# arpg/vicalib

Hardware: AMD Instinct MI355X
Metric: corner_residuals_per_sec (higher is better)
Workload: dtype f64

## Files before the change

### vicalib_amd/csrc/vc_imu.hpp

```cpp
#pragma once
#include "vc_math.hpp"

namespace vc {

struct D1 { double a, v; };
VC_HD D1 mk(double a, double v = 0.0) { D1 r; r.a = a; r.v = v; return r; }
VC_HD D1 operator+(D1 x, D1 y) { return mk(x.a + y.a, x.v + y.v); }
VC_HD D1 operator-(D1 x, D1 y) { return mk(x.a - y.a, x.v - y.v); }
VC_HD D1 operator-(D1 x) { return mk(-x.a, -x.v); }
VC_HD D1 operator*(D1 x, D1 y) { return mk(x.a * y.a, x.a * y.v + x.v * y.a); }
VC_HD D1 operator/(D1 x, D1 y) { const double inv = fast_rcp(y.a), q = x.a * inv; return mk(q, (x.v - q * y.v) * inv); }
VC_HD D1 operator+(D1 x, double s) { return mk(x.a + s, x.v); }
VC_HD D1 operator+(double s, D1 x) { return mk(x.a + s, x.v); }
VC_HD D1 operator-(D1 x, double s) { return mk(x.a - s, x.v); }
VC_HD D1 operator-(double s, D1 x) { return mk(s - x.a, -x.v); }
VC_HD D1 operator*(D1 x, double s) { return mk(x.a * s, x.v * s); }
VC_HD D1 operator*(double s, D1 x) { return mk(x.a * s, x.v * s); }
VC_HD D1 operator/(D1 x, double s) { const double inv = 1.0 / s; return mk(x.a * inv, x.v * inv); }
VC_HD D1 operator/(double s, D1 y) { const double inv = fast_rcp(y.a); return mk(s * inv, -s * inv * inv * y.v); }
VC_HD bool operator<(D1 x, double y) { return x.a < y; }
VC_HD bool operator>(D1 x, double y) { return x.a > y; }
VC_HD D1 sqrt(D1 x) { double s, is; fast_sqrt_rsqrt(x.a, &s, &is); return mk(s, 0.5 * x.v * is); }
VC_HD D1 sin(D1 x) { return mk(::sin(x.a), ::cos(x.a) * x.v); }
VC_HD D1 cos(D1 x) { return mk(::cos(x.a), -::sin(x.a) * x.v); }
// ... 304 lines not shown
  J[0 * 6 + 3] = 0.5 * q0; J[0 * 6 + 4] = -0.5 * q3; J[0 * 6 + 5] = 0.5 * q2;
  J[1 * 6 + 3] = 0.5 * q3; J[1 * 6 + 4] = 0.5 * q0; J[1 * 6 + 5] = -0.5 * q1;
  J[2 * 6 + 3] = -0.5 * q2; J[2 * 6 + 4] = 0.5 * q1; J[2 * 6 + 5] = 0.5 * q0;
  J[3 * 6 + 3] = -0.5 * q1; J[3 * 6 + 4] = -0.5 * q2; J[3 * 6 + 5] = -0.5 * q3;
  J[4 * 6 + 0] = 1.0 - 2.0 * (q2 * q2 + q3 * q3); J[4 * 6 + 1] = 2.0 * (q1 * q2 - q0 * q3); J[4 * 6 + 2] = 2.0 * (q1 * q3 + q0 * q2);
  J[5 * 6 + 0] = 2.0 * (q1 * q2 + q0 * q3); J[5 * 6 + 1] = 1.0 - 2.0 * (q1 * q1 + q3 * q3); J[5 * 6 + 2] = 2.0 * (q2 * q3 - q0 * q1);
  J[6 * 6 + 0] = 2.0 * (q1 * q3 - q0 * q2); J[6 * 6 + 1] = 2.0 * (q2 * q3 + q0 * q1); J[6 * 6 + 2] = 1.0 - 2.0 * (q1 * q1 + q2 * q2);
}

VC_HD void imu_block_direction(const ImuView& buf, double t_start, double t_end, const double* w_sqrt, int rotation_only,
                               const double* T2, const double* T1, const double* v2, const double* v1, const double* gdir,
                               const double* b, const double* sf, double toff, int dir, double* r, double* dr) {
  D1 P[35];
  for (int i = 0; i < 7; ++i) { P[i] = mk(T2[i]); P[7 + i] = mk(T1[i]); }
  for (int i = 0; i < 3; ++i) { P[14 + i] = mk(v2[i]); P[17 + i] = mk(v1[i]); }
  P[20] = mk(gdir[0]); P[21] = mk(gdir[1]);
  for (int i = 0; i < 6; ++i) { P[22 + i] = mk(b[i]); P[28 + i] = mk(sf[i]); }
  P[34] = mk(toff);
  for (int i = 0; i < 35; ++i) P[i].v = (i == dir) ? 1.0 : 0.0;
  D1 res[9];
  imu_residual<D1>(buf, t_start, t_end, w_sqrt, rotation_only, P, P + 7, P + 14, P + 17, P + 20, P + 22, P + 28, P[34], res);
  for (int i = 0; i < 9; ++i) { r[i] = res[i].a; dr[i] = res[i].v; }
}

constexpr int kDeltaCols = 14;

template <class T> struct DeltaAcc { T q[4], p[3], v[3], t; };
template <class T> VC_HD void imu_delta_append(DeltaAcc<T>* A, const PoseV<T>& d, T dt) {
  T rp[3], rv[3], q[4];
  tq_rotate(A->q, d.p, rp);
  tq_rotate(A->q, d.v, rv);
  tq_mul(A->q, d.q, q);
  for (int i = 0; i < 3; ++i) {
    A->p[i] = (A->p[i] + A->v[i] * dt) + rp[i];
    A->v[i] = A->v[i] + rv[i];
  }
  for (int i = 0; i < 4; ++i) A->q[i] = q[i];
  A->t = A->t + dt;
}
template <class T> VC_HD void imu_delta_then(DeltaAcc<T>* a, const DeltaAcc<T>& x) {
  PoseV<T> d;
  for (int k = 0; k < 4; ++k) d.q[k] = x.q[k];
  for (int k = 0; k < 3; ++k) { d.p[k] = x.p[k]; d.v[k] = x.v[k]; }
  imu_delta_append(a, d, x.t);
}
template <class T> VC_HD void imu_delta_identity(DeltaAcc<T>* a) {
  for (int k = 0; k < 3; ++k) { a->q[k] = cst<T>(0.0); a->p[k] = cst<T>(0.0); a->v[k] = cst<T>(0.0); }
  a->q[3] = cst<T>(1.0); a->t = cst<T>(0.0);
}
constexpr int kBlockDeltaStride = kDeltaCols * 11;

VC_HD void so3_exp_jl(const double* w, double* q, double* A, double* B) {
  const double th2 = w[0] * w[0] + w[1] * w[1] + w[2] * w[2];
  double imag, real;
  tso3_exp_factors(th2, &imag, &real);
  q[0] = imag * w[0]; q[1] = imag * w[1]; q[2] = imag * w[2]; q[3] = real;
  const bool tiny = th2 < 1e-6;
  *A = 2.0 * imag * imag;
  *B = tiny ? 1.0 / 6.0 - th2 * (1.0 / 120.0) : (1.0 - 2.0 * imag * real) * fast_rcp(tiny ? 1.0 : th2);
}
VC_HD void cross3(const double* a, const double* b, double* o) {
  const double x = a[1] * b[2] - a[2] * b[1], y = a[2] * b[0] - a[0] * b[2], z = a[0] * b[1] - a[1] * b[0];
  o[0] = x; o[1] = y; o[2] = z;
}
VC_HD void so3_jl_apply(const double* w, double A, double B, const double* d, double* o) {
  double c1[3], c2[3];
  cross3(w, d, c1);
  cross3(w, c1, c2);
  for (int i = 0; i < 3; ++i) o[i] = d[i] + A * c1[i] + B * c2[i];
}
VC_HD void mat3_vec(const double* R, const double* v, double* o) {
  const double a = R[0] * v[0] + R[1] * v[1] + R[2] * v[2];
  const double b = R[3] * v[0] + R[4] * v[1] + R[5] * v[2];
  const double c = R[6] * v[0] + R[7] * v[1] + R[8] * v[2];
  o[0] = a; o[1] = b; o[2] = c;
}
struct IntervalDeltaT { DeltaAcc<double> d; double dth[3], dp[3], dv[3], dt; double ap[3], av[3]; };
constexpr int kDtDoubles = 27;
VC_HD void imu_delta_t_identity(IntervalDeltaT* X) {
  imu_delta_identity(&X->d);
  for (int i = 0; i < 3; ++i) { X->dth[i] = 0.0; X->dp[i] = 0.0; X->dv[i] = 0.0; X->ap[i] = 0.0; X->av[i] = 0.0; }
  X->dt = 0.0;
}
VC_HD void imu_interval_delta_t(const ImuView& buf, const ImuRange& rg, D1 off, double t_start, double t_end, int m, int n_int,
                                const double* b, const double* sf, int gsel, IntervalDeltaT* X) {
  imu_delta_t_identity(X);
  const int kk = gsel < 3 ? gsel : (gsel < 6 ? gsel - 3 : 0);
  const bool seeded = gsel < 6, scale = gsel >= 3;
  double u0[3], u1[3], a0[3], a1[3], du0[3], du1[3], da0[3], da1[3], h, dh;
  double c0, c1;
  {
    Meas<D1> z0, z1;
    for (int k = 0; k < 3; ++k) { z0.w[k] = z0.a[k] = z1.w[k] = z1.a[k] = mk(0.0); }
    z0.time = z1.time = mk(0.0);
    if (m <= n_int) { imu_range_get_flat(buf, rg, off, t_start, t_end, m - 1, &z0); imu_range_get_flat(buf, rg, off, t_start, t_end, m, &z1); }
    if (z1.time.a == z0.time.a) return;
    h = z1.time.a - z0.time.a; dh = z1.time.v - z0.time.v;
    for (int i = 0; i < 3; ++i) {
      const double s0 = (seeded && i == kk) ? (scale ? z0.w[i].a : 1.0) : 0.0, s1 = (seeded && i == kk) ? (scale ? z1.w[i].a : 1.0) : 0.0;
      u0[i] = z0.w[i].a * sf[i] + b[i]; du0[i] = z0.w[i].v * sf[i] + s0;
      u1[i] = z1.w[i].a * sf[i] + b[i]; du1[i] = z1.w[i].v * sf[i] + s1;
      a0[i] = z0.a[i].a * sf[3 + i] + b[3 + i]; da0[i] = z0.a[i].v * sf[3 + i];
      a1[i] = z1.a[i].a * sf[3 + i] + b[3 + i]; da1[i] = z1.a[i].v * sf[3 + i];
    }
    c0 = scale ? (kk == 0 ? z0.a[0].a : kk == 1 ? z0.a[1].a : z0.a[2].a) : 1.0;
    c1 = scale ? (kk == 0 ? z1.a[0].a : kk == 1 ? z1.a[1].a : z1.a[2].a) : 1.0;
  }
  const double hh = h * 0.5, h6 = h / 6.0, dhh = dh * 0.5, dh6 = dh / 6.0;
  const double cm = 0.5 * c0 + 0.5 * c1;
  double sw[3], sv[3], sp[3], dsw[3], dsv[3], dsp[3], cv[3], cp[3], phi[3], dphi[3];
  for (int i = 0; i < 3; ++i) {
    sw[i] = u0[i]; dsw[i] = du0[i]; sv[i] = a0[i]; dsv[i] = da0[i]; sp[i] = a0[i]; dsp[i] = da0[i];
    cv[i] = (i == kk) ? c0 : 0.0; cp[i] = cv[i];
    phi[i] = u0[i] * hh; dphi[i] = du0[i] * hh + u0[i] * dhh;
  }
  for (int stage = 2; stage <= 4; ++stage) {
    double q[4], A, B, R[9], dth[3], ug[3], ua[3], dug[3], dua[3], wk[3], ak[3], dwk[3], dak[3], t1[3], t2[3];
    so3_exp_jl(phi, q, &A, &B);
    quat_to_R(q, R);
    so3_jl_apply(phi, A, B, dphi, dth);
    for (int i = 0; i < 3; ++i) {
      if (stage < 4) { ug[i] = u0[i] * 0.5 + u1[i] * 0.5; ua[i] = a0[i] * 0.5 + a1[i] * 0.5; dug[i] = du0[i] * 0.5 + du1[i] * 0.5; dua[i] = da0[i] * 0.5 + da1[i] * 0.5; }
      else { ug[i] = u1[i]; ua[i] = a1[i]; dug[i] = du1[i]; dua[i] = da1[i]; }
    }
    mat3_vec(R, ug, wk); mat3_vec(R, ua, ak);
    cross3(dth, wk, t1); mat3_vec(R, dug, t2);
    for (int i = 0; i < 3; ++i) dwk[i] = t1[i] + t2[i];
    cross3(dth, ak, t1); mat3_vec(R, dua, t2);
    for (int i = 0; i < 3; ++i) dak[i] = t1[i] + t2[i];
    const double r[3] = {kk == 0 ? R[0] : kk == 1 ? R[1] : R[2], kk == 0 ? R[3] : kk == 1 ? R[4] : R[5], kk == 0 ? R[6] : kk == 1 ? R[7] : R[8]};
    const double wgt = stage < 4 ? 2.0 : 1.0, cc = stage < 4 ? cm : c1;
    for (int i = 0; i < 3; ++i) {
      sw[i] = sw[i] + wgt * wk[i]; dsw[i] = dsw[i] + wgt * dwk[i];
      sv[i] = sv[i] + wgt * ak[i]; dsv[i] = dsv[i] + wgt * dak[i];
      cv[i] = cv[i] + wgt * (cc * r[i]);
      if (stage < 4) { sp[i] = sp[i] + ak[i]; dsp[i] = dsp[i] + dak[i]; cp[i] = cp[i] + cc * r[i]; }
      const double hs = stage == 2 ? hh : h, dhs = stage == 2 ? dhh : dh;
      if (stage < 4) { phi[i] = wk[i] * hs; dphi[i] = dwk[i] * hs + wk[i] * dhs; }
    }
  }
  {
    double A, B;
    for (int i = 0; i < 3; ++i) { phi[i] = sw[i] * h6; dphi[i] = dsw[i] * h6 + sw[i] * dh6; }
    so3_exp_jl(phi, X->d.q, &A, &B);
    so3_jl_apply(phi, A, B, dphi, X->dth);
    const double hh6 = h * h6, dhh6 = 2.0 * h * dh6;
    for (int i = 0; i < 3; ++i) {
      X->d.v[i] = sv[i] * h6; X->dv[i] = dsv[i] * h6 + sv[i] * dh6;
      X->d.p[i] = sp[i] * hh6; X->dp[i] = dsp[i] * hh6 + sp[i] * dhh6;
      X->av[i] = cv[i] * h6; X->ap[i] = cp[i] * hh6;
    }
    X->d.t = h; X->dt = dh;
  }
}
VC_HD void imu_delta_t_then(IntervalDeltaT* A, const IntervalDeltaT& X) {
  double R[9], rp[3], rv[3], t1[3], t2[3], t3[3], q[4];
  quat_to_R(A->d.q, R);
  mat3_vec(R, X.d.p, rp); mat3_vec(R, X.d.v, rv);
  cross3(A->dth, rp, t1); mat3_vec(R, X.dp, t2);
  for (int i = 0; i < 3; ++i) A->dp[i] = ((A->dp[i] + A->dv[i] * X.d.t) + A->d.v[i] * X.dt) + (t1[i] + t2[i]);
  cross3(A->dth, rv, t1); mat3_vec(R, X.dv, t2);
  for (int i = 0; i < 3; ++i) A->dv[i] = A->dv[i] + (t1[i] + t2[i]);
  mat3_vec(R, X.dth, t3);
  for (int i = 0; i < 3; ++i) A->dth[i] = A->dth[i] + t3[i];
  A->dt = A->dt + X.dt;
  mat3_vec(R, X.ap, t1); mat3_vec(R, X.av, t2);
  for (int i = 0; i < 3; ++i) {
    A->ap[i] = (A->ap[i] + A->av[i] * X.d.t) + t1[i];
    A->av[i] = A->av[i] + t2[i];
  }
  for (int i = 0; i < 3; ++i) {
    A->d.p[i] = (A->d.p[i] + A->d.v[i] * X.d.t) + rp[i];
    A->d.v[i] = A->d.v[i] + rv[i];
  }
  quat_mul(A->d.q, X.d.q, q);
  for (int i = 0; i < 4; ++i) A->d.q[i] = q[i];
  A->d.t = A->d.t + X.d.t;
}
VC_HD int imu_group_dual_col(int g) { return g < 3 ? 1 + g : (g < 6 ? 4 + g : 13); }
VC_HD int imu_group_accel_col(int g) { return g < 3 ? 4 + g : 7 + g; }
VC_HD void imu_block_record_store(const IntervalDeltaT& X, int g, double* rec) {
  if (g > 6) return;
  double* cd = rec + imu_group_dual_col(g) * 11;
  const double hq[4] = {0.5 * X.dth[0], 0.5 * X.dth[1], 0.5 * X.dth[2], 0.0};
  double dq[4];
  quat_mul(hq, X.d.q, dq);
  for (int k = 0; k < 4; ++k) cd[k] = dq[k];
  for (int k = 0; k < 3; ++k) { cd[4 + k] = X.dp[k]; cd[7 + k] = X.dv[k]; }
  cd[10] = X.dt;
  if (g < 6) {
    double* ca = rec + imu_group_accel_col(g) * 11;
    for (int k = 0; k < 4; ++k) ca[k] = 0.0;
    for (int k = 0; k < 3; ++k) { ca[4 + k] = X.ap[k]; ca[7 + k] = X.av[k]; }
    ca[10] = 0.0;
  }
  if (g == 0) {
    for (int k = 0; k < 4; ++k) rec[k] = X.d.q[k];
    for (int k = 0; k < 3; ++k) { rec[4 + k] = X.d.p[k]; rec[7 + k] = X.d.v[k]; }
    rec[10] = X.d.t;
  }
}
inline int imu_block_delta_record(const ImuView& buf, double t_start, double t_end, double toff, const double* b, const double* sf,
                                  double* rec ) {
  const ImuRange rg = imu_range(buf, t_start, t_end, toff);
  if (!rg.valid) { rec[10] = -1.0; return 0; }
  const int n_int = (rg.k1 - rg.k0 + 1) + 1;
  for (int g = 0; g < 7; ++g) {
    const D1 offD = mk(toff, g == 6 ? 1.0 : 0.0);
    IntervalDeltaT carry;
    for (int base = 0; base < n_int; base += 16) {
      IntervalDeltaT X[8], Y[8];
      for (int l = 0; l < 8; ++l) {
        IntervalDeltaT second;
        imu_interval_delta_t(buf, rg, offD, t_start, t_end, base + 2 * l + 1, n_int, b, sf, g, &X[l]);
        imu_interval_delta_t(buf, rg, offD, t_start, t_end, base + 2 * l + 2, n_int, b, sf, g, &second);
        imu_delta_t_then(&X[l], second);
      }
      for (int n = 1; n < 8; n <<= 1) {
        for (int l = 0; l < 8; ++l) { Y[l] = X[l]; if (l >= n) { Y[l] = X[l - n]; imu_delta_t_then(&Y[l], X[l]); } }
        for (int l = 0; l < 8; ++l) X[l] = Y[l];
      }
      if (base == 0) carry = X[7]; else imu_delta_t_then(&carry, X[7]);
    }
    imu_block_record_store(carry, g, rec);
  }
  return 1;
}

VC_HD void imu_block_final_direction(int valid, const double* block_rec, const double* w_sqrt, int rotation_only, const double* T2,
                                     const double* T1, const double* v2, const double* v1, const double* grav9 , int col,
                                     double* r, double* dr) {
  if (!valid) { for (int i = 0; i < 9; ++i) { r[i] = 0.0; dr[i] = 0.0; } return; }
  const int dcol = (col >= 20) ? col - 19 : 0;
  D1 Q[4], P[3], V[3];
  double bd[11];
  for (int k = 0; k < 11; ++k) { const double d = block_rec[dcol * 11 + k]; bd[k] = dcol ? d : 0.0; }
  for (int k = 0; k < 4; ++k) Q[k] = mk(block_rec[k], bd[k]);
  for (int k = 0; k < 3; ++k) { P[k] = mk(block_rec[4 + k], bd[4 + k]); V[k] = mk(block_rec[7 + k], bd[7 + k]); }
  const D1 Tt = mk(block_rec[10], bd[10]);
  D1 T2D[7], v2D[3], gw[3], q0[4], p0[3], v0[3];
  {
    double J[42];
    local_jac_se3(T2, J);
    for (int i = 0; i < 7; ++i) {
      double sel = 0.0;
      for (int c = 0; c < 6; ++c) sel = (col == c) ? J[i * 6 + c] : sel;
      T2D[i] = mk(T2[i], sel);
    }
    local_jac_se3(T1, J);
    for (int i = 0; i < 7; ++i) {
      double sel = 0.0;
      for (int c = 0; c < 6; ++c) sel = (col == 9 + c) ? J[i * 6 + c] : sel;
      if (i < 4) q0[i] = mk(T1[i], sel); else p0[i - 4] = mk(T1[i], sel);
    }
  }
  for (int k = 0; k < 3; ++k) { v2D[k] = mk(v2[k], col == 6 + k ? 1.0 : 0.0); v0[k] = mk(v1[k], col == 15 + k ? 1.0 : 0.0); }
  for (int k = 0; k < 3; ++k) gw[k] = mk(grav9[k], col == 18 ? grav9[3 + k] : (col == 19 ? grav9[6 + k] : 0.0));
  PoseV<D1> x;
  D1 rp[3], rv[3];
  tq_rotate(q0, P, rp);
  tq_rotate(q0, V, rv);
  tq_mul(q0, Q, x.q);
  const D1 ht2 = 0.5 * (Tt * Tt);
  for (int i = 0; i < 3; ++i) {
    x.p[i] = ((p0[i] + v0[i] * Tt) - gw[i] * ht2) + rp[i];
    x.v[i] = (v0[i] - gw[i] * Tt) + rv[i];
  }
  D1 res[9];
  imu_residual_tail(x, w_sqrt, rotation_only, T2D, v2D, res);
  for (int i = 0; i < 9; ++i) { r[i] = res[i].a; dr[i] = res[i].v; }
}

}
```

### vicalib_amd/csrc/vc_imu_kernels.hip

```cpp
#include <hip/hip_runtime.h>
#include <algorithm>
#include <cstdlib>
#include "vc_math.hpp"
#include "vc_imu.hpp"
#include "vc_imu_weights.hpp"
#include "vc_device.h"
#include "vc_kutil.hpp"
#include "vc_reduced_tail.hpp"
#include "vc_shared_blocks.hpp"

namespace vc {

__device__ __forceinline__ ImuView imu_view(const DevView& v) { ImuView b = {v.imu_t, v.imu_w, v.imu_a, v.n_imu, v.imu_avg_dt}; return b; }

constexpr int kImuJacLds = 34 * 9 + 6;
struct SegTab {
  unsigned short v[kSegStride];
  constexpr SegTab() : v() { for (int e = 0; e < kSegLen; ++e) { int a = 0, b = 0; seg_entry(e, &a, &b); v[e] = (unsigned short)(a | (b << 8)); } }
};
__constant__ SegTab d_seg_tab = SegTab();
constexpr int kSegIters = (kSegLen + 31) / 32;
#ifndef VC_IJ_MFMA
#define VC_IJ_MFMA 1
#endif
// ... 182 lines not shown
#pragma unroll
  for (int e = 0; e < N; ++e) x[e] += y[e];
}
template <int N> __device__ __forceinline__ void row_allsum_n(double* x) {
  row_add_level<0xB1, N>(x);
  row_add_level<0x4E, N>(x);
  row_add_level<0x141, N>(x);
  row_add_level<0x140, N>(x);
}
__device__ __forceinline__ double shfl16(double x, int src) { return __shfl(x, src, 16); }
__device__ __forceinline__ void delta_identity(DeltaAcc<double>* a) {
#pragma unroll
  for (int k = 0; k < 3; ++k) { a->q[k] = 0.0; a->p[k] = 0.0; a->v[k] = 0.0; }
  a->q[3] = 1.0; a->t = 0.0;
}
__device__ __forceinline__ void delta_then(DeltaAcc<double>* a, const DeltaAcc<double>& x) {
  PoseV<double> d;
#pragma unroll
  for (int k = 0; k < 4; ++k) d.q[k] = x.q[k];
#pragma unroll
  for (int k = 0; k < 3; ++k) { d.p[k] = x.p[k]; d.v[k] = x.v[k]; }
  imu_delta_append(a, d, x.t);
}
template <int N> __device__ __forceinline__ void delta_scan_level(DeltaAcc<double>* X, int c) {
  DeltaAcc<double> A;
#pragma unroll
  for (int k = 0; k < 4; ++k) A.q[k] = row_shr<N>(X->q[k], X->q[k]);
#pragma unroll
  for (int k = 0; k < 3; ++k) { A.p[k] = row_shr<N>(X->p[k], X->p[k]); A.v[k] = row_shr<N>(X->v[k], X->v[k]); }
  A.t = row_shr<N>(X->t, X->t);
  delta_then(&A, *X);
  if (c >= N) *X = A;
}
template <int N> __device__ __forceinline__ void map_scan_level(double* S) {
  double B[kWMapF], O[kWMapF];
  w_map_identity(B);
#pragma unroll
  for (int e = 0; e < kWMapF; ++e) B[e] = row_shl<N>(B[e], S[e]);
  w_map_compose(B, S, O);
#pragma unroll
  for (int e = 0; e < kWMapF; ++e) S[e] = O[e];
}

__device__ __forceinline__ ImuRange imu_range_lanes(const ImuView& b, double t0, double t1, double off, int lane) {
  ImuRange r; r.valid = 0; r.k0 = 0; r.k1 = -1; r.i0 = r.i1 = 0; r.first_end = r.last_end = 0;
  if (b.n < 2) return r;
  const bool odd = lane & 1;
  int idx, endc, le;
  imu_element_index(b, odd ? t1 : t0, off, &idx, &endc, &le);
  const int idx_o = __shfl_xor(idx, 1, 64), endc_o = __shfl_xor(endc, 1, 64), le_o = __shfl_xor(le, 1, 64);
  r.valid = (t0 >= b.t[0] + off && t0 <= b.t[b.n - 1] + off) ? 1 : 0;
  r.i0 = odd ? idx_o : idx; r.first_end = odd ? endc_o : endc;
  r.i1 = odd ? idx : idx_o; r.last_end = odd ? endc : endc_o;
  r.k0 = r.i0 + 1;
  r.k1 = odd ? le : le_o;
  if (r.k1 < r.i0) r.k1 = r.i0;
  return r;
}

__device__ __forceinline__ void delta_t_pack(const IntervalDeltaT& X, double* f) {
#pragma unroll
  for (int k = 0; k < 4; ++k) f[k] = X.d.q[k];
#pragma unroll
  for (int k = 0; k < 3; ++k) { f[4 + k] = X.d.p[k]; f[7 + k] = X.d.v[k]; f[11 + k] = X.dth[k]; f[14 + k] = X.dp[k]; f[17 + k] = X.dv[k]; f[21 + k] = X.ap[k]; f[24 + k] = X.av[k]; }
  f[10] = X.d.t; f[20] = X.dt;
}
__device__ __forceinline__ void delta_t_unpack(const double* f, IntervalDeltaT* X) {
#pragma unroll
  for (int k = 0; k < 4; ++k) X->d.q[k] = f[k];
#pragma unroll
  for (int k = 0; k < 3; ++k) { X->d.p[k] = f[4 + k]; X->d.v[k] = f[7 + k]; X->dth[k] = f[11 + k]; X->dp[k] = f[14 + k]; X->dv[k] = f[17 + k]; X->ap[k] = f[21 + k]; X->av[k] = f[24 + k]; }
  X->d.t = f[10]; X->dt = f[20];
}
template <int N> __device__ __forceinline__ void delta_t_scan_level(IntervalDeltaT* X, int l) {
  double f[kDtDoubles];
  delta_t_pack(*X, f);
#pragma unroll
  for (int k = 0; k < kDtDoubles; ++k) f[k] = row_shr<N>(f[k], f[k]);
  IntervalDeltaT A;
  delta_t_unpack(f, &A);
  imu_delta_t_then(&A, *X);
  if (l >= N) *X = A;
}
#ifdef VC_IB_STAMPS
#define IBSTAMP(i) do { if (blockIdx.x == gridDim.x / 2 && threadIdx.x == 0) v.dbg[i] = (long long)__builtin_amdgcn_s_memrealtime(); } while (0)
#else
#define IBSTAMP(i) do { } while (0)
#endif
#ifndef VC_IMU_BLOCK_WAVES
#define VC_IMU_BLOCK_WAVES 2
#endif
#ifdef VC_IMU_BLOCK_EU
__global__ __launch_bounds__(256) __attribute__((amdgpu_waves_per_eu(VC_IMU_BLOCK_EU, VC_IMU_BLOCK_EU))) void k_imu_block(DevView v, int trial) {
#else
__global__ __launch_bounds__(256, VC_IMU_BLOCK_WAVES) void k_imu_block(DevView v, int trial) {
#endif
  __shared__ double s_carry[32 * kDtDoubles];
  __shared__ double s_park[256 * (kDtDoubles - 11)];
  __shared__ double s_parkv[4 * 8 * 11];
  IBSTAMP(0);
  if (trial && v.sync_seq > 0 && workgroup_pass_void(v)) return;
  const int lane = threadIdx.x & 63, wave = __builtin_amdgcn_readfirstlane(threadIdx.x >> 6);
  const int g = lane >> 3, l = lane & 7;
  const int n_blocks = v.n_frames - 1;
  const int s_raw = blockIdx.x * 4 + wave;
  const int s = s_raw < n_blocks ? s_raw : n_blocks - 1;
  const double toff0 = v.imus[0][14], toff1 = v.imus[1][14];
  const double t_start = v.frame_time[s], t_end = v.frame_time[s + 1];
  const Ctrl* ct = v.ctrl;
  const int c_done = ct->done, c_need = ct->need_lin, c_cur = ct->cur;
  if (c_done || (!trial && !c_need)) return;
  IBSTAMP(1);
  const int cur = trial ? 1 - c_cur : c_cur;
  const double* im = v.imus[cur];
  const double toff = cur ? toff1 : toff0;
  const ImuView buf = imu_view(v);
  ImuRange rg = imu_range_lanes(buf, t_start, t_end, toff, lane);
  rg.valid = __builtin_amdgcn_readfirstlane(rg.valid); rg.i0 = __builtin_amdgcn_readfirstlane(rg.i0); rg.i1 = __builtin_amdgcn_readfirstlane(rg.i1);
  rg.k0 = __builtin_amdgcn_readfirstlane(rg.k0); rg.k1 = __builtin_amdgcn_readfirstlane(rg.k1);
  rg.first_end = __builtin_amdgcn_readfirstlane(rg.first_end); rg.last_end = __builtin_amdgcn_readfirstlane(rg.last_end);
  double* rec = v.imu_delta_blk + (size_t)s * kBlockDeltaStride;
  IBSTAMP(2);
  if (rg.valid) {
    const int n_int = (rg.k1 - rg.k0 + 1) + 1;
    const int gsel = g < 7 ? g : 6;
    double* cr = s_carry + (threadIdx.x >> 3) * kDtDoubles;
    IntervalDeltaT X;
#pragma unroll 1
    for (int base = 0; base < n_int; base += 16) {
      {
        IntervalDeltaT Y;
        double* pk = s_park + threadIdx.x;
        double* pv = s_parkv + (wave * 8 + l) * 11;
#pragma unroll 1
        for (int half = 0; half < 2; ++half) {
          int gs = gsel;
          asm volatile("" : "+v"(gs));
          imu_interval_delta_t(buf, rg, mk(toff, gs == 6 ? 1.0 : 0.0), t_start, t_end, base + 2 * l + 1 + half, n_int, im + 2, im + 8, gs, &Y);
          IBSTAMP(3 + half);
          if (half == 0) {
            double f[kDtDoubles];
            delta_t_pack(Y, f);
#pragma unroll
            for (int k = 11; k < kDtDoubles; ++k) pk[(k - 11) * 256] = f[k];
            if (g == 0) {
#pragma unroll
              for (int k = 0; k < 11; ++k) pv[k] = f[k];
            }
          }
        }
        wave_lds_sync_local();
        double f[kDtDoubles];
#pragma unroll
        for (int k = 0; k < 11; ++k) f[k] = pv[k];
#pragma unroll
        for (int k = 11; k < kDtDoubles; ++k) f[k] = pk[(k - 11) * 256];
        delta_t_unpack(f, &X);
        wave_lds_sync_local();
        imu_delta_t_then(&X, Y);
      }
      IBSTAMP(5);
      delta_t_scan_level<1>(&X, l); delta_t_scan_level<2>(&X, l); delta_t_scan_level<4>(&X, l);
      IBSTAMP(6);
      if (l == 7) {
        if (base > 0) {
          IntervalDeltaT A;
          double f[kDtDoubles];
#pragma unroll
          for (int k = 0; k < kDtDoubles; ++k) f[k] = cr[k];
          delta_t_unpack(f, &A);
          imu_delta_t_then(&A, X);
          X = A;
        }
        if (base + 16 < n_int) {
          double f[kDtDoubles];
          delta_t_pack(X, f);
#pragma unroll
          for (int k = 0; k < kDtDoubles; ++k) cr[k] = f[k];
        }
      }
    }
    if (l == 7 && s_raw < n_blocks) imu_block_record_store(X, g, rec);
    IBSTAMP(7);
  } else if (lane == 0 && s_raw < n_blocks) rec[10] = -1.0;
  if (blockIdx.x == 0 && threadIdx.x == 63) imu_gravity_record(im, v.imu_grav + cur * 16);
  if (trial && v.block_wait > 0 && blockIdx.x == 0 && threadIdx.x == 0) spin_until_flag<false>(v, 2, v.block_wait);
}

#ifdef VC_W_STAMPS
#define WSTAMP(i) do { if (blockIdx.x == 0 && threadIdx.x == 0) v.dbg[i] = (long long)__builtin_amdgcn_s_memrealtime(); } while (0)
#else
#define WSTAMP(i) do { } while (0)
#endif
__global__ __launch_bounds__(64) void k_imu_weights(DevView v, int wr) {
  __shared__ __attribute__((aligned(16))) double w_lds[4 * kWLds];
  const Ctrl* ct = v.ctrl;
  const int lane = threadIdx.x;
  const int grp = lane >> 4, c = lane & 15;
  const int n_blocks = v.n_frames - 1;
  const int s_raw = blockIdx.x * 4 + grp;
  const bool exists = s_raw < n_blocks;
  const int s = exists ? s_raw : n_blocks - 1;
  double* L = w_lds + grp * kWLds;
  if (v.sync_seq > 0) { const long long m = sync_marked(v); if (m != 0 && m <= v.sync_seq) return; }
  if (ct->done == kDoneSyncTimeout) return;
  if (ct->done || !v.weights_on) {
    if (exists) for (int e = c; e < 81; e += 16) v.wsqrtb[1 - wr][(size_t)s * 81 + e] = v.wsqrtb[wr][(size_t)s * 81 + e];
    return;
  }
  WSTAMP(0);
  const int j = s + 1;
  {
    const double p0 = v.poses[0][(size_t)(j - 1) * kPoseStride + c], p1 = v.poses[1][(size_t)(j - 1) * kPoseStride + c];
    const double u0 = v.vel[0][(size_t)(j - 1) * 4 + (c & 3)], u1 = v.vel[1][(size_t)(j - 1) * 4 + (c & 3)];
    const int ci = c < 15 ? c : 14;
    const double i0 = v.imus[0][ci], i1 = v.imus[1][ci];
    const bool one = ct->cur != 0;
    L[kWPose + c] = one ? p1 : p0;
    if (c < 4) L[kWVel + c] = one ? u1 : u0;
    if (c < 15) L[kWImu + c] = one ? i1 : i0;
  }
  const double t_start = v.frame_time[j - 1], t_end = v.frame_time[j];
  wave_lds_sync();
  double b[6], sf[6];
#pragma unroll
  for (int i = 0; i < 6; ++i) { b[i] = L[kWImu + 2 + i]; sf[i] = L[kWImu + 8 + i]; }
  const double toff = L[kWImu + 14];
  const ImuView buf = imu_view(v);
  const ImuRange rg = imu_range_lanes(buf, t_start, t_end, toff, lane);
  const bool live = exists && rg.valid;
  const double sg2 = v.gyro_sigma * v.gyro_sigma, sa2 = v.accel_sigma * v.accel_sigma;
  const int n_int = live ? (rg.k1 - rg.k0 + 1) + 1 : 0;
  int n_max = n_int;
#pragma unroll
  for (int o = 32; o >= 16; o >>= 1) n_max = max(n_max, __shfl_xor(n_max, o, 64));
  DeltaAcc<double> carry;
  delta_identity(&carry);
  const double g0[3] = {0.0, 0.0, 0.0};
  WSTAMP(1);
#pragma unroll 1
  for (int base = 0; base < n_max; base += 16) {
    const int m = base + c + 1;
    Meas<double> z0, z1;
#pragma unroll
    for (int k = 0; k < 3; ++k) { z0.w[k] = z0.a[k] = z1.w[k] = z1.a[k] = 0.0; }
    z0.time = z1.time = 0.0;
    if (m <= n_int) { imu_range_get_flat(buf, rg, toff, t_start, t_end, m - 1, &z0); imu_range_get_flat(buf, rg, toff, t_start, t_end, m, &z1); }
    const bool act = z1.time != z0.time;
    WSTAMP(2);
    DeltaAcc<double> X;
    {
      PoseV<double> d;
#pragma unroll
      for (int k = 0; k < 3; ++k) { d.q[k] = 0.0; d.p[k] = 0.0; d.v[k] = 0.0; }
      d.q[3] = 1.0;
      imu_rk4_step(&d, z0, z1, b, sf, g0);
#pragma unroll
      for (int k = 0; k < 4; ++k) X.q[k] = d.q[k];
#pragma unroll
      for (int k = 0; k < 3; ++k) { X.p[k] = d.p[k]; X.v[k] = d.v[k]; }
      X.t = z1.time - z0.time;
    }
    WSTAMP(3);
    delta_scan_level<1>(&X, c); delta_scan_level<2>(&X, c); delta_scan_level<4>(&X, c); delta_scan_level<8>(&X, c);
    double q_st[4];
    {
      double qe[4], ident[4] = {0.0, 0.0, 0.0, 1.0};
// ... 2169 lines not shown
#pragma unroll
      for (int u = 0; u < NL; ++u) {
        const unsigned qf = (unsigned)(row * 57) >> 9;
        const bool masked = (mbits >> qf) & 1u;
        tmp[u] = (row < nrow && !masked) ? src[(unsigned)(row * v.ldx + col) + qf * skip] : 0.0;
        row += step_r; col += step_c;
        if (col >= ld) { col -= ld; ++row; }
      }
    };
    request(f0);
    for (int fg = f0; fg < f1; fg += 4) {
#pragma unroll
      for (int u = 0; u < NL; ++u) { const int i = tid + 256 * u; if (i < 36 * ld) R[i] = tmp[u]; }
      __syncthreads();
      GSTAMP(gs_); ++gs_;
      if (fg + 4 < f1) request(fg + 4);
      const double* rq = R + (lane >> 4) * ld + (lane & 15);
      int oa[NQ], ob[NQ];
#pragma unroll
      for (int q = 0; q < NQ; ++q) {
        const int p = min(pb + 4 * q + wave, nPairs - 1);
        const int ij = s_pair[p];
        oa[q] = (ij & 255) * 16; ob[q] = (ij >> 8) * 16;
      }
#pragma unroll
      for (int ks = 0; ks < 9; ++ks)
#pragma unroll
        for (int q = 0; q < NQ; ++q) acc[q] = __builtin_amdgcn_mfma_f64_16x16x4f64(rq[ks * 4 * ld + oa[q]], rq[ks * 4 * ld + ob[q]], acc[q], 0, 0, 0);
      __syncthreads();
      GSTAMP(gs_); ++gs_;
    }
#pragma unroll
    for (int q = 0; q < NQ; ++q) {
      const int p = pb + 4 * q + wave;
      if (p < nPairs) {
        const int ij = s_pair[p], I = ij & 255, J = ij >> 8;
#pragma unroll
        for (int g = 0; g < 4; ++g) {
          const int row = I * 16 + (lane >> 4) + 4 * g, col = J * 16 + (lane & 15);
          if (row < D && col <= D) {
            double* dst = col < D ? part + row * D + col : part + D * D + row;
            if (publish) __hip_atomic_store(dst, acc[q][g], __ATOMIC_RELAXED, __HIP_MEMORY_SCOPE_AGENT); else *dst = acc[q][g];
          }
        }
      }
    }
  }
  if (publish) {
    __builtin_amdgcn_s_waitcnt(0);
    __syncthreads();
    if (tid == 0) __hip_atomic_store(v.part_ready + chunk, v.pass_id, __ATOMIC_RELAXED, __HIP_MEMORY_SCOPE_AGENT);
  }
#ifdef VC_GRAM_STAMPS
  __builtin_amdgcn_s_waitcnt(0);
  GSTAMP(15);
#endif
}
template <int NQ, int NL>
__global__ __launch_bounds__(256, 2) void k_chain_gram(DevView v, int gather) {
  extern __shared__ __attribute__((aligned(16))) double R[];
  __shared__ unsigned short s_pair[128];
  if (gather) chain_gram_chunk<NQ, NL>(v, v.n_chunks, R, s_pair, 0, v.gram_top_stride);
  else chain_gram_chunk<NQ, NL>(v, (int)blockIdx.x, R, s_pair, v.gram_top_stride);
}
template <int NW, int NQ, int NL>
__global__ __launch_bounds__(256) void k_chain_top_gram(DevView v, int s, int m, int lvl) {
  extern __shared__ __attribute__((aligned(16))) double R[];
  __shared__ unsigned short s_pair[128];
  __shared__ __attribute__((aligned(16))) double XS[9 * kXsLd];
  __shared__ double An[81];
  __shared__ double Ls_all[NW * 81];
  if (blockIdx.x == 0) {
    if ((int)threadIdx.x >= 64 * NW) return;
    chain_fwd_group<1, NW>(v, s, m, 1, lvl, 0, (int)(threadIdx.x >> 6), XS, An, Ls_all);
    return;
  }
  if ((int)blockIdx.x == 1 + v.n_chunks) { hadd_side_job(v, R, 256); return; }
  if ((int)blockIdx.x > 1 + v.n_chunks) { part_sum_ride_job(v, (int)blockIdx.x - 2 - v.n_chunks, R); return; }
  chain_gram_chunk<NQ, NL>(v, (int)blockIdx.x - 1, R, s_pair, v.gram_top_stride, 0, v.part_ride != 0);
}

void launch_imu_delta(const DevView& v, hipStream_t s, int trial) {
  if (v.n_frames < 2) return;
  hipLaunchKernelGGL(k_imu_block, dim3((v.n_frames - 1 + 3) / 4), dim3(256), 0, s, v, trial);
}
void launch_imu_jac(const DevView& v, int wr, hipStream_t s, int trial) {
  if (v.n_frames < 2) return;
  hipLaunchKernelGGL(k_imu_jac, dim3((v.n_frames - 1 + 7) / 8), dim3(256), 0, s, v, wr, trial);
}
void launch_imu_weights(const DevView& v, int wr, hipStream_t s) {
  if (v.n_frames < 2) return;
  hipLaunchKernelGGL(k_imu_weights, dim3((v.n_frames - 1 + 3) / 4), dim3(64), 0, s, v, wr);
}
void launch_chain_gram(const DevView& v, hipStream_t s);
static void chain_levels(const DevView& v, const ChainPlan& p, hipStream_t s, bool forward) {
  const int N = v.n_frames;
  if (N < 1) return;
  const int nl = p.n_levels, top_stride = p.top_stride, m_top = kChainM;
  const int cpl = (v.D + 1 + 27 + 63) / 64;
  auto fwd = [&](int groups, int stride, int m, int top, int lvl) {
    if (!top && p.two[lvl]) {
      const int extra = (v.hadd_early && lvl == 1) ? (v.part_stride - (v.D * v.D + v.D) + 15) / 16 : 0;
      if (cpl <= 1) hipLaunchKernelGGL(k_chain_fwd2<1>, dim3(groups + extra), dim3(128), 0, s, v, stride, m, lvl, groups);
      else hipLaunchKernelGGL(k_chain_fwd2<2>, dim3(groups + extra), dim3(256), 0, s, v, stride, m, lvl, groups);
    }
    else if (cpl <= 1) hipLaunchKernelGGL((k_chain_fwd<1, 1>), dim3(groups), dim3(64), 0, s, v, stride, m, top, lvl);
    else if (cpl <= 2) hipLaunchKernelGGL((k_chain_fwd<1, 2>), dim3(groups), dim3(128), 0, s, v, stride, m, top, lvl);
    else if (cpl <= 3) hipLaunchKernelGGL((k_chain_fwd<1, 3>), dim3(groups), dim3(192), 0, s, v, stride, m, top, lvl);
    else hipLaunchKernelGGL((k_chain_fwd<1, 4>), dim3(groups), dim3(256), 0, s, v, stride, m, top, lvl);
  };
  if (forward) {
    for (int l = 0; l < nl; ++l) {
      if (l == 0 && v.fold_l0) {
        if (v.n_cams <= 1) hipLaunchKernelGGL(k_chain_l0<1>, dim3(p.groups[0]), dim3(256), 0, s, v);
        else hipLaunchKernelGGL(k_chain_l0<2>, dim3(p.groups[0]), dim3(256), 0, s, v);
      } else fwd(p.groups[l], p.stride[l], p.m[l], 0, l);
    }
    if (v.gram_top_stride > 0) {
      const size_t lds = std::max((size_t)36 * v.ldw, (size_t)(v.hadd_early ? kHaddLds : 0)) * sizeof(double);
      const int ride_blocks = (v.part_ride && v.hadd_early) ? (v.D * v.D + v.D + 15) / 16 : 0;
      const int nT = (v.D + 1 + 15) / 16, nPairs = nT * (nT + 1) / 2, nq = std::min(kMaxPairsPerWaveI, (nPairs + 3) / 4);
      const int nlr = (36 * v.ldw + 255) / 256;
      auto go = [&](auto kern) {
        if (lds > 40000) (void)hipFuncSetAttribute((const void*)kern, hipFuncAttributeMaxDynamicSharedMemorySize, (int)lds);
        hipLaunchKernelGGL(kern, dim3(1 + v.n_chunks + (v.hadd_early ? 1 : 0) + ride_blocks), dim3(256), lds, s, v, top_stride, m_top, nl);
      };
      if (cpl <= 1) { if (nq <= 1) go(k_chain_top_gram<1, 1, 7>); else go(k_chain_top_gram<1, 2, 7>); }
      else if (cpl <= 2) { if (nlr <= 12) go(k_chain_top_gram<2, 4, 12>); else if (nq <= 6) go(k_chain_top_gram<2, 6, 16>); else go(k_chain_top_gram<2, 9, 16>); }
      else if (cpl <= 3) { if (nlr <= 16) go(k_chain_top_gram<3, 9, 16>); else if (nlr <= 21) go(k_chain_top_gram<3, 9, 21>); else go(k_chain_top_gram<3, 9, 25>); }
      else { if (nlr <= 25) go(k_chain_top_gram<4, 9, 25>); else go(k_chain_top_gram<4, 9, 30>); }
    } else {
      fwd(1, top_stride, m_top, 1, nl);
    }
  } else {
    if (v.back_path && nl >= 1 && nl <= 5) {
      BackPath P; P.n = nl;
      for (int l = 0; l < 6; ++l) { P.stride[l] = l < nl ? p.stride[l] : 1; P.m[l] = l < nl ? p.m[l] : 2; P.two[l] = l < nl ? p.two[l] : 0; }
      const bool ct0 = v.D + 1 > kPathRowCols;
      P.top_stride = top_stride; P.ldr = ct0 ? 1 : ((v.D + 1) | 1); P.dsw = ((v.D + 63) / 64) * 64;
      if (ct0) hipLaunchKernelGGL(k_chain_t0, dim3((N + 3) / 4), dim3(256), 0, s, v);
      const int nw = nl + 1;
      P.tail = (v.tail_deferred && nw >= 4) ? 1 : 0;
      const size_t lds = std::max(((size_t)nw * kPathDl + (size_t)nw * P.dsw + 4 + (ct0 ? 0 : (size_t)nw * 63 * P.ldr)), (size_t)(P.tail ? kTailLds : 0)) * sizeof(double);
      static LdsGrant g4, g6;
      auto go = [&](auto kern, LdsGrant& g) {
        if (lds > 60000 && g.need(lds)) (void)hipFuncSetAttribute((const void*)kern, hipFuncAttributeMaxDynamicSharedMemorySize, (int)lds);
        hipLaunchKernelGGL(kern, dim3(p.groups[0] + P.tail), dim3(64 * nw), lds, s, v, P);
      };
      if (nw <= 4) { if (ct0) go(k_chain_back_path<4, true>, g4); else go(k_chain_back_path<4, false>, g4); }
      else { if (ct0) go(k_chain_back_path<6, true>, g6); else go(k_chain_back_path<6, false>, g6); }
      return;
    }
    hipLaunchKernelGGL(k_chain_back, dim3(1 + (nl > 0 ? (N + kBackT0Frames - 1) / kBackT0Frames : 0)), dim3(64), 0, s, v, top_stride, m_top, 1, nl, 0);
    int total_groups = 0;
    for (int l = 0; l < nl; ++l) total_groups += p.groups[l];
    static const int resident_limit = [] {
      int dev = 0, per_cu = 0; hipDeviceProp_t pr;
      if (hipGetDevice(&dev) != hipSuccess || hipGetDeviceProperties(&pr, dev) != hipSuccess ||
          hipOccupancyMaxActiveBlocksPerMultiprocessor(&per_cu, (const void*)k_chain_back_levels, 64, 0) != hipSuccess || per_cu <= 0) return 2048;
      return std::max(64, per_cu * pr.multiProcessorCount / 2);
    }();
    if (nl > 0 && nl <= 8 && v.cready && total_groups <= resident_limit) {
      BackLevels L; L.n = nl;
      int at = 0;
      for (int i = 0; i < nl; ++i) {
        const int l = nl - 1 - i;
        L.start[i] = at; L.stride[i] = p.stride[l]; L.m[i] = p.m[l]; L.two[i] = p.two[l];
// ... 40 lines not shown
```

Before: 2.114 billion.

## Pack two IMU blocks per wave with shared element staging and serial-4 scan

Restructures k_imu_block so each wave handles two inter-frame blocks (32 lanes each, 8 gradient groups by 4 lanes) instead of one, halving the grid. IMU range elements are fetched once into LDS and reused by all gradient groups rather than re-interpolated per lane, and the time-offset derivative is only carried for the time-offset column. Each lane now composes four intervals serially and the scan shrinks to two levels. This trades more sequential work per lane and extra LDS syncs for fewer redundant measurement loads and better lane utilisation. The host reference path is updated to the same grouping.

New measurement: 2.116 billion (median of 6 runs). Within noise of the previous version (+0.1%).

```diff
diff --git a/vicalib_amd/csrc/vc_imu.hpp b/vicalib_amd/csrc/vc_imu.hpp
--- a/vicalib_amd/csrc/vc_imu.hpp
+++ b/vicalib_amd/csrc/vc_imu.hpp
@@ -410,26 +410,28 @@
   for (int i = 0; i < 3; ++i) { X->dth[i] = 0.0; X->dp[i] = 0.0; X->dv[i] = 0.0; X->ap[i] = 0.0; X->av[i] = 0.0; }
   X->dt = 0.0;
 }
-VC_HD void imu_interval_delta_t(const ImuView& buf, const ImuRange& rg, D1 off, double t_start, double t_end, int m, int n_int,
-                                const double* b, const double* sf, int gsel, IntervalDeltaT* X) {
+VC_HD void imu_range_element_t(const ImuView& buf, const ImuRange& rg, double toff, double t_start, double t_end, int which, Meas<D1>* z) {
+  imu_range_get_flat(buf, rg, mk(toff, 1.0), t_start, t_end, which, z);
+}
+VC_HD void imu_interval_delta_t(const Meas<D1>& z0, const Meas<D1>& z1, bool live, const double* b, const double* sf, int gsel,
+                                IntervalDeltaT* X) {
   imu_delta_t_identity(X);
   const int kk = gsel < 3 ? gsel : (gsel < 6 ? gsel - 3 : 0);
   const bool seeded = gsel < 6, scale = gsel >= 3;
   double u0[3], u1[3], a0[3], a1[3], du0[3], du1[3], da0[3], da1[3], h, dh;
   double c0, c1;
   {
-    Meas<D1> z0, z1;
-    for (int k = 0; k < 3; ++k) { z0.w[k] = z0.a[k] = z1.w[k] = z1.a[k] = mk(0.0); }
-    z0.time = z1.time = mk(0.0);
-    if (m <= n_int) { imu_range_get_flat(buf, rg, off, t_start, t_end, m - 1, &z0); imu_range_get_flat(buf, rg, off, t_start, t_end, m, &z1); }
-    if (z1.time.a == z0.time.a) return;
-    h = z1.time.a - z0.time.a; dh = z1.time.v - z0.time.v;
+    const double t0 = live ? z0.time.a : 0.0, t1 = live ? z1.time.a : 0.0;
+    if (t1 == t0) return;
+    const bool tv = !seeded;
+    h = t1 - t0; dh = tv ? z1.time.v - z0.time.v : 0.0;
     for (int i = 0; i < 3; ++i) {
       const double s0 = (seeded && i == kk) ? (scale ? z0.w[i].a : 1.0) : 0.0, s1 = (seeded && i == kk) ? (scale ? z1.w[i].a : 1.0) : 0.0;
-      u0[i] = z0.w[i].a * sf[i] + b[i]; du0[i] = z0.w[i].v * sf[i] + s0;
-      u1[i] = z1.w[i].a * sf[i] + b[i]; du1[i] = z1.w[i].v * sf[i] + s1;
-      a0[i] = z0.a[i].a * sf[3 + i] + b[3 + i]; da0[i] = z0.a[i].v * sf[3 + i];
-      a1[i] = z1.a[i].a * sf[3 + i] + b[3 + i]; da1[i] = z1.a[i].v * sf[3 + i];
+      const double w0v = tv ? z0.w[i].v : 0.0, w1v = tv ? z1.w[i].v : 0.0, a0v = tv ? z0.a[i].v : 0.0, a1v = tv ? z1.a[i].v : 0.0;
+      u0[i] = z0.w[i].a * sf[i] + b[i]; du0[i] = w0v * sf[i] + s0;
+      u1[i] = z1.w[i].a * sf[i] + b[i]; du1[i] = w1v * sf[i] + s1;
+      a0[i] = z0.a[i].a * sf[3 + i] + b[3 + i]; da0[i] = a0v * sf[3 + i];
+      a1[i] = z1.a[i].a * sf[3 + i] + b[3 + i]; da1[i] = a1v * sf[3 + i];
     }
     c0 = scale ? (kk == 0 ? z0.a[0].a : kk == 1 ? z0.a[1].a : z0.a[2].a) : 1.0;
     c1 = scale ? (kk == 0 ? z1.a[0].a : kk == 1 ? z1.a[1].a : z1.a[2].a) : 1.0;
@@ -534,21 +536,27 @@
   if (!rg.valid) { rec[10] = -1.0; return 0; }
   const int n_int = (rg.k1 - rg.k0 + 1) + 1;
   for (int g = 0; g < 7; ++g) {
-    const D1 offD = mk(toff, g == 6 ? 1.0 : 0.0);
     IntervalDeltaT carry;
     for (int base = 0; base < n_int; base += 16) {
-      IntervalDeltaT X[8], Y[8];
-      for (int l = 0; l < 8; ++l) {
-        IntervalDeltaT second;
-        imu_interval_delta_t(buf, rg, offD, t_start, t_end, base + 2 * l + 1, n_int, b, sf, g, &X[l]);
-        imu_interval_delta_t(buf, rg, offD, t_start, t_end, base + 2 * l + 2, n_int, b, sf, g, &second);
-        imu_delta_t_then(&X[l], second);
+      IntervalDeltaT X[4], Y[4];
+      for (int l = 0; l < 4; ++l) {
+        for (int k = 0; k < 4; ++k) {
+          const int m = base + 4 * l + k + 1;
+          const bool live = m <= n_int;
+          Meas<D1> z0, z1;
+          for (int i = 0; i < 3; ++i) { z0.w[i] = z0.a[i] = z1.w[i] = z1.a[i] = mk(0.0); }
+          z0.time = z1.time = mk(0.0);
+          if (live) { imu_range_element_t(buf, rg, toff, t_start, t_end, m - 1, &z0); imu_range_element_t(buf, rg, toff, t_start, t_end, m, &z1); }
+          IntervalDeltaT step;
+          imu_interval_delta_t(z0, z1, live, b, sf, g, &step);
+          if (k == 0) X[l] = step; else imu_delta_t_then(&X[l], step);
+        }
       }
-      for (int n = 1; n < 8; n <<= 1) {
-        for (int l = 0; l < 8; ++l) { Y[l] = X[l]; if (l >= n) { Y[l] = X[l - n]; imu_delta_t_then(&Y[l], X[l]); } }
-        for (int l = 0; l < 8; ++l) X[l] = Y[l];
+      for (int n = 1; n < 4; n <<= 1) {
+        for (int l = 0; l < 4; ++l) { Y[l] = X[l]; if (l >= n) { Y[l] = X[l - n]; imu_delta_t_then(&Y[l], X[l]); } }
+        for (int l = 0; l < 4; ++l) X[l] = Y[l];
       }
-      if (base == 0) carry = X[7]; else imu_delta_t_then(&carry, X[7]);
+      if (base == 0) carry = X[3]; else imu_delta_t_then(&carry, X[3]);
     }
     imu_block_record_store(carry, g, rec);
   }
diff --git a/vicalib_amd/csrc/vc_imu_kernels.hip b/vicalib_amd/csrc/vc_imu_kernels.hip
--- a/vicalib_amd/csrc/vc_imu_kernels.hip
+++ b/vicalib_amd/csrc/vc_imu_kernels.hip
@@ -288,29 +288,52 @@
   imu_delta_t_then(&A, *X);
   if (l >= N) *X = A;
 }
+__device__ __forceinline__ void park_put(const IntervalDeltaT& X, bool values, double* gv, double* gt, int st) {
+  double f[kDtDoubles];
+  delta_t_pack(X, f);
+#pragma unroll
+  for (int k = 11; k < kDtDoubles; ++k) gt[(k - 11) * st] = f[k];
+  if (values) {
+#pragma unroll
+    for (int k = 0; k < 11; ++k) gv[k] = f[k];
+  }
+}
+__device__ __forceinline__ void park_get(const double* gv, const double* gt, int st, IntervalDeltaT* X) {
+  double f[kDtDoubles];
+#pragma unroll
+  for (int k = 0; k < 11; ++k) f[k] = gv[k];
+#pragma unroll
+  for (int k = 11; k < kDtDoubles; ++k) f[k] = gt[(k - 11) * st];
+  delta_t_unpack(f, X);
+}
+struct IbLane { int tid, half, g, l, hb; };
+__device__ __forceinline__ IbLane ib_lane() {
+  int t = threadIdx.x;
+  asm volatile("" : "+v"(t));
+  IbLane r; r.tid = t; r.half = (t >> 5) & 1; r.g = (t >> 2) & 7; r.l = t & 3; r.hb = t >> 5;
+  return r;
+}
+constexpr int kIbElems = 17;
+constexpr int kIbElemD = 14;
 #ifdef VC_IB_STAMPS
 #define IBSTAMP(i) do { if (blockIdx.x == gridDim.x / 2 && threadIdx.x == 0) v.dbg[i] = (long long)__builtin_amdgcn_s_memrealtime(); } while (0)
 #else
 #define IBSTAMP(i) do { } while (0)
 #endif
-#ifndef VC_IMU_BLOCK_WAVES
-#define VC_IMU_BLOCK_WAVES 2
-#endif
-#ifdef VC_IMU_BLOCK_EU
-__global__ __launch_bounds__(256) __attribute__((amdgpu_waves_per_eu(VC_IMU_BLOCK_EU, VC_IMU_BLOCK_EU))) void k_imu_block(DevView v, int trial) {
-#else
-__global__ __launch_bounds__(256, VC_IMU_BLOCK_WAVES) void k_imu_block(DevView v, int trial) {
-#endif
-  __shared__ double s_carry[32 * kDtDoubles];
+__global__ __launch_bounds__(256, 2) void k_imu_block(DevView v, int trial) {
+  __shared__ double s_elem[8 * kIbElems * kIbElemD];
   __shared__ double s_park[256 * (kDtDoubles - 11)];
-  __shared__ double s_parkv[4 * 8 * 11];
+  __shared__ double s_parkv[8 * 4 * 11];
+  __shared__ double s_carry[64 * (kDtDoubles - 11)];
+  __shared__ double s_carryv[8 * 11];
   IBSTAMP(0);
   if (trial && v.sync_seq > 0 && workgroup_pass_void(v)) return;
   const int lane = threadIdx.x & 63, wave = __builtin_amdgcn_readfirstlane(threadIdx.x >> 6);
-  const int g = lane >> 3, l = lane & 7;
+  const int half = lane >> 5;
   const int n_blocks = v.n_frames - 1;
-  const int s_raw = blockIdx.x * 4 + wave;
-  const int s = s_raw < n_blocks ? s_raw : n_blocks - 1;
+  const int s_raw = (blockIdx.x * 4 + wave) * 2 + half;
+  const bool exists = s_raw < n_blocks;
+  const int s = exists ? s_raw : n_blocks - 1;
   const double toff0 = v.imus[0][14], toff1 = v.imus[1][14];
   const double t_start = v.frame_time[s], t_end = v.frame_time[s + 1];
   const Ctrl* ct = v.ctrl;
@@ -321,74 +344,97 @@
   const double* im = v.imus[cur];
   const double toff = cur ? toff1 : toff0;
   const ImuView buf = imu_view(v);
-  ImuRange rg = imu_range_lanes(buf, t_start, t_end, toff, lane);
-  rg.valid = __builtin_amdgcn_readfirstlane(rg.valid); rg.i0 = __builtin_amdgcn_readfirstlane(rg.i0); rg.i1 = __builtin_amdgcn_readfirstlane(rg.i1);
-  rg.k0 = __builtin_amdgcn_readfirstlane(rg.k0); rg.k1 = __builtin_amdgcn_readfirstlane(rg.k1);
-  rg.first_end = __builtin_amdgcn_readfirstlane(rg.first_end); rg.last_end = __builtin_amdgcn_readfirstlane(rg.last_end);
-  double* rec = v.imu_delta_blk + (size_t)s * kBlockDeltaStride;
+  ImuRange rgs[2];
+  double ts[2], te[2];
+  int ni[2];
+  {
+    const ImuRange rg = imu_range_lanes(buf, t_start, t_end, toff, lane);
+#pragma unroll
+    for (int h = 0; h < 2; ++h) {
+      rgs[h].valid = __builtin_amdgcn_readlane(rg.valid, 32 * h); rgs[h].i0 = __builtin_amdgcn_readlane(rg.i0, 32 * h);
+      rgs[h].i1 = __builtin_amdgcn_readlane(rg.i1, 32 * h); rgs[h].k0 = __builtin_amdgcn_readlane(rg.k0, 32 * h);
+      rgs[h].k1 = __builtin_amdgcn_readlane(rg.k1, 32 * h); rgs[h].first_end = __builtin_amdgcn_readlane(rg.first_end, 32 * h);
+      rgs[h].last_end = __builtin_amdgcn_readlane(rg.last_end, 32 * h);
+      ts[h] = readlane_f64(t_start, 32 * h); te[h] = readlane_f64(t_end, 32 * h);
+      ni[h] = rgs[h].valid ? (rgs[h].k1 - rgs[h].k0 + 1) + 1 : 0;
+    }
+  }
+  const int n_max = max(ni[0], ni[1]);
   IBSTAMP(2);
-  if (rg.valid) {
-    const int n_int = (rg.k1 - rg.k0 + 1) + 1;
-    const int gsel = g < 7 ? g : 6;
-    double* cr = s_carry + (threadIdx.x >> 3) * kDtDoubles;
-    IntervalDeltaT X;
 #pragma unroll 1
-    for (int base = 0; base < n_int; base += 16) {
+  for (int base = 0; base < n_max; base += 16) {
+    {
+      const IbLane q = ib_lane();
+      const int n_int = q.half ? ni[1] : ni[0];
+      const int e_ld = q.g < 4 ? 4 * q.l + q.g : 16;
+      if ((q.g < 4 || (q.g == 4 && q.l == 3)) && base + e_ld <= n_int) {
+        const ImuRange rg = q.half ? rgs[1] : rgs[0];
+        Meas<D1> z;
+        imu_range_element_t(buf, rg, toff, q.half ? ts[1] : ts[0], q.half ? te[1] : te[0], base + e_ld, &z);
+        double* d = s_elem + (q.hb * kIbElems + e_ld) * kIbElemD;
+#pragma unroll
+        for (int k = 0; k < 3; ++k) { d[k] = z.w[k].a; d[3 + k] = z.a[k].a; d[7 + k] = z.w[k].v; d[10 + k] = z.a[k].v; }
+        d[6] = z.time.a; d[13] = z.time.v;
+      }
+    }
+    wave_lds_sync_local();
+    IBSTAMP(3);
+    IntervalDeltaT Y;
+#pragma unroll 1
+    for (int k = 0; k < 4; ++k) {
       {
-        IntervalDeltaT Y;
-        double* pk = s_park + threadIdx.x;
-        double* pv = s_parkv + (wave * 8 + l) * 11;
-#pragma unroll 1
-        for (int half = 0; half < 2; ++half) {
-          int gs = gsel;
-          asm volatile("" : "+v"(gs));
-          imu_interval_delta_t(buf, rg, mk(toff, gs == 6 ? 1.0 : 0.0), t_start, t_end, base + 2 * l + 1 + half, n_int, im + 2, im + 8, gs, &Y);
-          IBSTAMP(3 + half);
-          if (half == 0) {
-            double f[kDtDoubles];
-            delta_t_pack(Y, f);
-#pragma unroll
-            for (int k = 11; k < kDtDoubles; ++k) pk[(k - 11) * 256] = f[k];
-            if (g == 0) {
-#pragma unroll
-              for (int k = 0; k < 11; ++k) pv[k] = f[k];
-            }
-          }
+        const IbLane q = ib_lane();
+        const int m = base + 4 * q.l + k + 1;
+        const bool live = m <= (q.half ? ni[1] : ni[0]);
+        Meas<D1> z0, z1;
+        const double* d0 = s_elem + (q.hb * kIbElems + 4 * q.l + k) * kIbElemD;
+        const double* d1 = d0 + kIbElemD;
+#pragma unroll
+        for (int i = 0; i < 3; ++i) {
+          z0.w[i] = mk(d0[i], d0[7 + i]); z0.a[i] = mk(d0[3 + i], d0[10 + i]);
+          z1.w[i] = mk(d1[i], d1[7 + i]); z1.a[i] = mk(d1[3 + i], d1[10 + i]);
         }
-        wave_lds_sync_local();
-        double f[kDtDoubles];
-#pragma unroll
-        for (int k = 0; k < 11; ++k) f[k] = pv[k];
-#pragma unroll
-        for (int k = 11; k < kDtDoubles; ++k) f[k] = pk[(k - 11) * 256];
-        delta_t_unpack(f, &X);
-        wave_lds_sync_local();
+        z0.time = mk(d0[6], d0[13]); z1.time = mk(d1[6], d1[13]);
+        imu_interval_delta_t(z0, z1, live, im + 2, im + 8, q.g < 7 ? q.g : 6, &Y);
+      }
+      if (k == 0) IBSTAMP(4);
+      const IbLane q = ib_lane();
+      double* pt = s_park + q.tid;
+      double* pv = s_parkv + (q.hb * 4 + q.l) * 11;
+      if (k > 0) {
+        IntervalDeltaT X;
+        park_get(pv, pt, 256, &X);
         imu_delta_t_then(&X, Y);
-      }
-      IBSTAMP(5);
-      delta_t_scan_level<1>(&X, l); delta_t_scan_level<2>(&X, l); delta_t_scan_level<4>(&X, l);
-      IBSTAMP(6);
-      if (l == 7) {
+        Y = X;
+      }
+      if (k < 3) park_put(Y, q.g == 0, pv, pt, 256);
+      wave_lds_sync_local();
+    }
+    IBSTAMP(5);
+    IntervalDeltaT X = Y;
+    delta_t_scan_level<1>(&X, threadIdx.x & 3); delta_t_scan_level<2>(&X, threadIdx.x & 3);
+    IBSTAMP(6);
+    {
+      const IbLane q = ib_lane();
+      const int n_int = q.half ? ni[1] : ni[0];
+      if (q.l == 3 && base < n_int) {
+        double* cr = s_carry + (q.tid >> 2);
+        double* cv = s_carryv + q.hb * 11;
         if (base > 0) {
           IntervalDeltaT A;
-          double f[kDtDoubles];
-#pragma unroll
-          for (int k = 0; k < kDtDoubles; ++k) f[k] = cr[k];
-          delta_t_unpack(f, &A);
+          park_get(cv, cr, 64, &A);
           imu_delta_t_then(&A, X);
           X = A;
         }
-        if (base + 16 < n_int) {
-          double f[kDtDoubles];
-          delta_t_pack(X, f);
-#pragma unroll
-          for (int k = 0; k < kDtDoubles; ++k) cr[k] = f[k];
-        }
-      }
-    }
-    if (l == 7 && s_raw < n_blocks) imu_block_record_store(X, g, rec);
-    IBSTAMP(7);
-  } else if (lane == 0 && s_raw < n_blocks) rec[10] = -1.0;
+        const int sr = blockIdx.x * 8 + q.hb;
+        if (base + 16 < n_int) park_put(X, q.g == 0, cv, cr, 64);
+        else if (sr < n_blocks) imu_block_record_store(X, q.g, v.imu_delta_blk + (size_t)sr * kBlockDeltaStride);
+      }
+    }
+    wave_lds_sync_local();
+  }
+  IBSTAMP(7);
+  if ((half ? ni[1] : ni[0]) == 0 && exists && (lane & 31) == 0) v.imu_delta_blk[(size_t)s * kBlockDeltaStride + 10] = -1.0;
   if (blockIdx.x == 0 && threadIdx.x == 63) imu_gravity_record(im, v.imu_grav + cur * 16);
   if (trial && v.block_wait > 0 && blockIdx.x == 0 && threadIdx.x == 0) spin_until_flag<false>(v, 2, v.block_wait);
 }
@@ -2724,7 +2770,7 @@
 
 void launch_imu_delta(const DevView& v, hipStream_t s, int trial) {
   if (v.n_frames < 2) return;
-  hipLaunchKernelGGL(k_imu_block, dim3((v.n_frames - 1 + 3) / 4), dim3(256), 0, s, v, trial);
+  hipLaunchKernelGGL(k_imu_block, dim3((v.n_frames - 1 + 7) / 8), dim3(256), 0, s, v, trial);
 }
 void launch_imu_jac(const DevView& v, int wr, hipStream_t s, int trial) {
   if (v.n_frames < 2) return;
```
